# LemonATsu/UNet-PhaseGen

Measured on NVIDIA B200. Metric: audio_seconds_per_second_mag_to_phase_to_wave, higher is better.
Workload: dtype f16x3/f16x2/f16-fp32acc (two-product fp16 on d1,u2; single fp16 product = TF32 operand rounding on u1)

## Files before the change

### unet-phasegen_b200/csrc/api.cu

```cuda
#include <cstdarg>
#include <cstdio>

#include "common.cuh"
#include "conv_plan.h"

namespace pg {
static thread_local char g_err[512] = "";

void set_error(const char* fmt, ...) {
    va_list ap;
    va_start(ap, fmt);
    vsnprintf(g_err, sizeof(g_err), fmt, ap);
    va_end(ap);
}

int check_launch(const char* what) {
    cudaError_t e = cudaGetLastError();
    if (e != cudaSuccess) {
        set_error("%s: launch failed: %s", what, cudaGetErrorString(e));
        return PG_ERR_CUDA;
    }
    return PG_OK;
}
}
// ... 26 lines not shown
    pg::ConvPlan pl;
    int rc = pg::conv_plan_build(d, &pl);
    if (rc != PG_OK) return rc;
    return pl.OS * pl.n_ntiles;
}

extern "C" int pg_conv_tc_plan(const pg_conv_desc* d, int* out, int n_out) {
    PG_REQUIRE(d && out && n_out >= 16, "pg_conv_tc_plan: need a descriptor and room for 16 ints");
    pg::ConvPlan p;
    int rc = pg::conv_plan_build(d, &p);
    if (rc != PG_OK) return rc;
    const int v[16] = {p.n_tile, p.n_ntiles, p.nb, p.strip_rows, p.pair, p.merged, p.mgroups, p.acc_stages,
                       p.n_chunks, p.n_cotiles, p.OS, p.IS, p.n_taps[0], p.n_taps[1], p.n_groups[0], p.n_groups[1]};
    for (int i = 0; i < 16; ++i) out[i] = v[i];
    if (n_out >= 17) out[16] = p.whole_clip;
    return PG_OK;
}
```

### unet-phasegen_b200/csrc/conv_plan.h

```cpp
#pragma once
#include <stdint.h>
#include <stdlib.h>

#include "../../include/phasegen.h"
#include "common.cuh"

namespace pg {

constexpr int kMaxTaps = 32;

struct ConvTap { int8_t w_idx; int8_t shift; int8_t parity; int8_t pad_; int32_t d; };
struct ConvGroup { int32_t row0; int8_t parity; int8_t n_taps; int8_t first_tap; int8_t pad_; };

struct ConvPlan {
    int B, C_in, C_out, L_in, L_out, k;
    int IS, OS;
    int n_tile, n_ntiles;
    int n_chunks, n_cotiles;
    int strip_rows;
    int nb;
    int acc_stages;
    int pair;
    int mgroups;
    int merged;
    int clip_group;
    int whole_clip;
    int out_rows, out_ld;
    int n_groups[2], n_taps[2];
    ConvGroup groups[2][kMaxTaps];
    ConvTap taps[2][kMaxTaps];
};

static inline int floordiv(int a, int b) { return (a >= 0) ? a / b : -((-a + b - 1) / b); }

static inline int conv_plan_build(const pg_conv_desc* d, ConvPlan* p) {
    const int s = d->stride, k = d->k, pad = d->pad;
    if (s < 1 || s > 2 || k < 1 || k > kMaxTaps) { set_error("conv plan: stride must be 1 or 2 and k <= %d (got s=%d k=%d)", kMaxTaps, s, k); return PG_ERR_UNSUPPORTED; }
    const bool tr = d->kind == PG_CONV_TRANSPOSE;
    const int L_expect = tr ? (d->L_in - 1) * s - 2 * pad + k : (d->L_in + 2 * pad - k) / s + 1;
    const bool len_ok = tr ? (d->L_out >= L_expect && d->L_out < L_expect + s) : d->L_out == L_expect;
    if (!len_ok || d->L_out < 1) { set_error("conv plan: L_out %d does not match geometry (expected %d)", d->L_out, L_expect); return PG_ERR_INVALID; }
// ... 122 lines not shown
                const int planes = (d->precision == PG_PREC_BF16X3 || d->precision == PG_PREC_F16X3 || d->precision == PG_PREC_F16X2) ? 2 : 1;
                if (nb * p->n_ntiles * p->strip_rows * planes * 128 > 72 * 1024) nb = 1;
                if (p->n_ntiles * p->strip_rows * planes * 128 > 80 * 1024) {
                    set_error("conv plan: the %d strips of a whole clip (%d rows each) do not fit shared memory", p->n_ntiles, p->strip_rows);
                    return PG_ERR_UNSUPPORTED;
                }
                p->nb = nb;
            }
        }
    }
    {
        const int cols = p->merged ? p->nb * p->strip_rows : p->nb * p->n_tile * (p->whole_clip ? p->OS * p->n_ntiles : 1);
        if (cols > 512) { set_error("conv plan: tile needs %d accumulator columns (> 512)", cols); return PG_ERR_UNSUPPORTED; }
        p->acc_stages = cols <= 256 ? 2 : 1;
    }
    p->clip_group = d->B;
    return PG_OK;
}

}
```

### unet-phasegen_b200/csrc/conv_tc.cu

```cuda
#include "tc_ptx.cuh"
#include "conv_plan.h"

namespace pg {

struct ConvTcParams {
    ConvPlan plan;
    float* y;
    float4* stats;
    int n_a_slots;
    int b_slot_bytes;
    int n_terms;
    int f16;
    int base_offset_mode;
    int a_mn;
    int epi_mode;
    const float* gamma; const float* beta; float eps;
    ActDst dst0, dst1;
    float2* ss_out;
    const int* clip_rows;
};

constexpr int kThreads = 192;
constexpr int kATileBytes = 128 * 128;
constexpr int kMaxASlots = 8;

struct TileCoord { int co_tile, phase, b0, nt; };

__device__ __forceinline__ int n_bundles(const ConvPlan& p) { return (p.B + p.nb - 1) / p.nb; }
__device__ __forceinline__ int n_co_slabs(const ConvPlan& p) { return p.pair ? p.n_cotiles / 2 : p.n_cotiles; }
__device__ __forceinline__ int tile_OS(const ConvPlan& p) { return p.whole_clip ? 1 : p.OS; }
__device__ __forceinline__ int tile_NT(const ConvPlan& p) { return p.whole_clip ? 1 : p.n_ntiles; }
__device__ __forceinline__ int total_tiles(const ConvPlan& p) { return n_co_slabs(p) * tile_OS(p) * n_bundles(p) * tile_NT(p); }
__device__ __forceinline__ TileCoord decode_tile(const ConvPlan& p, int tile) {
    TileCoord c;
    const int OSx = tile_OS(p), NTx = tile_NT(p);
    const int nbg = n_bundles(p), G = p.clip_group, n_slabs = n_co_slabs(p) * OSx;
    const int tiles_full = n_slabs * G * NTx;
    const int g = tile / tiles_full, r = tile % tiles_full;
    int Gg = nbg - g * G; if (Gg > G) Gg = G;
    const int per_slab = Gg * NTx;
    const int slab = r / per_slab, r2 = r % per_slab;
    c.co_tile = slab / OSx; c.phase = slab % OSx;
    c.b0 = (g * G + r2 / NTx) * p.nb; c.nt = r2 % NTx;
    return c;
}

template <bool PAIR, bool RAGGED>
__global__ void __launch_bounds__(kThreads, 1)
conv_tc_kernel(const __grid_constant__ CUtensorMap map_w_hi, const __grid_constant__ CUtensorMap map_w_lo,
               const __grid_constant__ CUtensorMap map_x_hi, const __grid_constant__ CUtensorMap map_x_lo,
               const __grid_constant__ ConvTcParams prm) {
    extern __shared__ __align__(1024) uint8_t smem_raw[];
    const ConvPlan& pl = prm.plan;
    uint8_t* smem = reinterpret_cast<uint8_t*>((reinterpret_cast<uintptr_t>(smem_raw) + 1023) & ~uintptr_t(1023));
    const int nA = prm.n_a_slots;
    const int bPlane = prm.b_slot_bytes;
    const int a_planes = prm.n_terms == 3 ? 2 : 1;
    const int b_planes = prm.n_terms >= 2 ? 2 : 1;
    uint8_t* a_base = smem;
    uint8_t* b_base = a_base + (size_t)nA * a_planes * kATileBytes;
    uint64_t* bars = reinterpret_cast<uint64_t*>(b_base + 2 * (size_t)b_planes * bPlane);
    uint64_t* fullA = bars;
    uint64_t* emptyA = bars + kMaxASlots;
    uint64_t* fullB = bars + 2 * kMaxASlots;
    uint64_t* emptyB = fullB + 2;
    uint64_t* accFull = emptyB + 2;
    uint64_t* accEmpty = accFull + 2;
    uint32_t* tmem_slot = reinterpret_cast<uint32_t*>(accEmpty + 2);
    uint32_t* epi_tiles = reinterpret_cast<uint32_t*>(reinterpret_cast<uint8_t*>(bars) + 256);

    const int warp = __shfl_sync(0xffffffffu, (int)(threadIdx.x >> 5), 0), lane = threadIdx.x & 31;
    const int n_tiles = total_tiles(pl);
    const bool w_lo = prm.n_terms == 3, x_lo = prm.n_terms >= 2;

    if (warp == 0 && lane == 0) {
        tma_prefetch_desc(&map_w_hi); tma_prefetch_desc(&map_x_hi);
        if (w_lo) tma_prefetch_desc(&map_w_lo);
        if (x_lo) tma_prefetch_desc(&map_x_lo);
        for (int i = 0; i < nA; ++i) { mbar_init(fullA + i, 1); mbar_init(emptyA + i, 1); }
        for (int i = 0; i < 2; ++i) {
            mbar_init(fullB + i, 1); mbar_init(emptyB + i, 1);
            mbar_init(accFull + i, 1); mbar_init(accEmpty + i, PAIR ? 8 : 4);
        }
        fence_barrier_init();
    }
    if (warp == 1) { if (PAIR) tmem_alloc_pair(tmem_slot, 512); else tmem_alloc(tmem_slot, 512); }
    tc_fence_before();
    if (PAIR) cluster_sync_all(); else __syncthreads();
    tc_fence_after();
    const uint32_t tmem_base = __shfl_sync(0xffffffffu, *tmem_slot, 0);
    const int rank = PAIR ? (int)cluster_ctarank() : 0;
    const int tile0 = PAIR ? (int)(blockIdx.x >> 1) : (int)blockIdx.x;
    const int tile_step = PAIR ? (int)(gridDim.x >> 1) : (int)gridDim.x;
    const int half_n = pl.n_tile >> 1;
    const int nb_grp = pl.nb / pl.mgroups;
    const int nb_cta = (PAIR && pl.merged) ? nb_grp >> 1 : nb_grp;
    const int t_phases = pl.whole_clip ? pl.OS : 1;
    const int t_nts = pl.whole_clip ? pl.n_ntiles : 1;
    const int n_sub = pl.merged ? pl.mgroups : t_nts;

    if (warp == 0) {
        {
            uint32_t b_it = 0;
            int a_slot = 0; uint32_t a_ph = 0;
            const uint32_t grp_bytes = (uint32_t)nb_cta * pl.strip_rows * 128u;
            const uint32_t a_bytes = a_planes * kATileBytes;
            const uint32_t b_bytes = b_planes * (uint32_t)bPlane;
            for (int tile = tile0; tile < n_tiles; tile += tile_step) {
                TileCoord tc = decode_tile(pl, tile);
                if (PAIR) tc.co_tile = tc.co_tile * 2 + rank;
                const int m0 = tc.nt * pl.n_tile + ((PAIR && !pl.merged) ? rank * half_n : 0);
                const int clip0 = tc.b0 + ((PAIR && pl.merged) ? rank * nb_cta : 0);
                for (int ch = 0; ch < pl.n_chunks; ++ch) {
                  for (int ph = tc.phase; ph < tc.phase + t_phases; ++ph) {
                    const int ng = pl.n_groups[ph];
                    for (int g = 0; g < ng; ++g) {
                        const ConvGroup grp = pl.groups[ph][g];
                        {
                            const int s = b_it & 1; const uint32_t bph = (b_it >> 1) & 1;
                            mbar_wait(emptyB + s, bph ^ 1);
                            uint8_t* dst = b_base + (size_t)s * b_planes * bPlane;
                            if (elect_one()) {
                                if (PAIR) { if (rank == 0) mbar_expect_tx(fullB + s, 2 * b_bytes); }
                                else mbar_expect_tx(fullB + s, b_bytes);
                                for (int sub = 0; sub < n_sub; ++sub) {
                                    uint8_t* dg = dst + (size_t)sub * grp_bytes;
                                    const int cg = clip0 + (pl.merged ? sub * nb_grp : 0);
                                    const int r0 = m0 + (pl.merged ? 0 : sub * pl.n_tile) + grp.row0;
                                    if (PAIR) {
                                        tma_load_4d_pair(dg, &map_x_hi, fullB + s, ch * 64, grp.parity, r0, cg);
                                        if (x_lo) tma_load_4d_pair(dg + bPlane, &map_x_lo, fullB + s, ch * 64, grp.parity, r0, cg);
                                    } else {
                                        tma_load_4d(dg, &map_x_hi, fullB + s, ch * 64, grp.parity, r0, cg);
                                        if (x_lo) tma_load_4d(dg + bPlane, &map_x_lo, fullB + s, ch * 64, grp.parity, r0, cg);
                                    }
                                }
                            }
                            __syncwarp();
                            ++b_it;
                        }
                        for (int j = 0; j < grp.n_taps; ++j) {
                            const int w_idx = pl.taps[ph][grp.first_tap + j].w_idx;
                            const int s = a_slot; const uint32_t aph = a_ph;
                            mbar_wait(emptyA + s, aph ^ 1);
                            uint8_t* dst = a_base + (size_t)s * a_planes * kATileBytes;
                            if (elect_one()) {
                                if (!PAIR) mbar_expect_tx(fullA + s, a_bytes);
                                else if (rank == 0) mbar_expect_tx(fullA + s, 2 * a_bytes);
                                auto load_w = [&](uint8_t* d, const CUtensorMap* m, int c0, int c1) {
                                    if (PAIR) tma_load_3d_pair(d, m, fullA + s, c0, c1, w_idx);
                                    else tma_load_3d(d, m, fullA + s, c0, c1, w_idx);
                                };
                                if (prm.a_mn) {
                                    for (int h = 0; h < 2; ++h) {
                                        load_w(dst + h * 8192, &map_w_hi, tc.co_tile * 128 + h * 64, ch * 64);
                                        if (w_lo) load_w(dst + kATileBytes + h * 8192, &map_w_lo, tc.co_tile * 128 + h * 64, ch * 64);
                                    }
                                } else {
                                    load_w(dst, &map_w_hi, ch * 64, tc.co_tile * 128);
                                    if (w_lo) load_w(dst + kATileBytes, &map_w_lo, ch * 64, tc.co_tile * 128);
                                }
                            }
                            __syncwarp();
                            if (++a_slot == nA) { a_slot = 0; a_ph ^= 1; }
                        }
                    }
                  }
                }
            }
        }
    } else if (warp == 1) {
        if (rank == 0) {
            uint32_t b_it = 0, t_it = 0;
            int a_slot = 0; uint32_t a_ph = 0;
            const int n_mma = pl.merged ? nb_grp * pl.strip_rows : pl.n_tile;
            const int n_outer = pl.merged ? 1 : t_nts, n_inner = pl.merged ? pl.mgroups : pl.nb;
            const uint32_t dcol_step = pl.merged ? (uint32_t)n_mma : (uint32_t)(pl.n_tile * t_phases * t_nts);
            const uint32_t idesc = (make_idesc_bf16(n_mma, PAIR ? 256 : 128) & ~(prm.f16 ? ((7u << 7) | (7u << 10)) : 0u)) |
                                   (prm.a_mn ? (1u << 15) : 0u);
            const bool a_mn = prm.a_mn != 0;
            auto mma = [&](uint32_t d, uint32_t da, uint32_t db, uint32_t acc_flag) {
                if (elect_one()) { if (PAIR) umma_words_pair(d, da, db, idesc, acc_flag); else umma_words(d, da, db, idesc, acc_flag); }
            };
            const uint32_t a_step = a_mn ? (2048u >> 4) : (32u >> 4);
            auto commit = [&](uint64_t* bar) {
                if (elect_one()) { if (PAIR) umma_commit_pair(bar); else umma_commit(bar); }
                __syncwarp();
            };
            for (int tile = tile0; tile < n_tiles; tile += tile_step, ++t_it) {
                TileCoord tc = decode_tile(pl, tile);
                const int acc = pl.acc_stages == 2 ? (t_it & 1) : 0;
                const uint32_t acc_ph = pl.acc_stages == 2 ? ((t_it >> 1) & 1) : (t_it & 1);
                mbar_wait_sleep(accEmpty + acc, acc_ph ^ 1, 200);
                tc_fence_after();
                const uint32_t d_tmem = tmem_base + acc * 256;
                const uint32_t strip_bytes = (uint32_t)pl.strip_rows * 128u;
                const uint32_t clip_step = (pl.merged ? (uint32_t)nb_cta * strip_bytes : strip_bytes) >> 4;
                for (int ch = 0; ch < pl.n_chunks; ++ch) {
                  for (int ph = tc.phase; ph < tc.phase + t_phases; ++ph) {
                    const int ng = pl.n_groups[ph];
                    const uint32_t dcol_ph = d_tmem + (uint32_t)((ph - tc.phase) * t_nts * pl.n_tile);
                    for (int g = 0; g < ng; ++g) {
                        const ConvGroup grp = pl.groups[ph][g];
                        const int bs = b_it & 1; const uint32_t bph = (b_it >> 1) & 1;
                        mbar_wait(fullB + bs, bph);
                        tc_fence_after();
                        const uint32_t b_hi = smem_u32(b_base + (size_t)bs * b_planes * bPlane);
// ... 20 lines not shown
                                            mma(dcol, aw_hi + kk * a_step, bw_lo + kk * 2, 1);
                                            mma(dcol, aw_hi + kk * a_step, bw_hi + kk * 2, 1);
                                        }
                                    } else if (x_lo) {
#pragma unroll
                                        for (uint32_t kk = 0; kk < 4; ++kk) {
                                            mma(dcol, aw_hi + kk * a_step, bw_lo + kk * 2, kk == 0 ? acc_first : 1u);
                                            mma(dcol, aw_hi + kk * a_step, bw_hi + kk * 2, 1);
                                        }
                                    } else {
#pragma unroll
                                        for (uint32_t kk = 0; kk < 4; ++kk) mma(dcol, aw_hi + kk * a_step, bw_hi + kk * 2, kk == 0 ? acc_first : 1u);
                                    }
                                }
                            }
                            commit(emptyA + as);
                            if (++a_slot == nA) { a_slot = 0; a_ph ^= 1; }
                        }
                        commit(emptyB + bs);
                        ++b_it;
                    }
                  }
                }
                commit(accFull + acc);
            }
        }
    } else {
        const int q = warp & 3;
        uint32_t* tile = epi_tiles + q * 512;
        uint32_t t_it = 0;
        const int n_parts = t_phases * t_nts;
        const int col_pitch = pl.merged ? pl.strip_rows : pl.n_tile * n_parts;
        bool bad_range = false;
        auto store_f32 = [&](float* base, size_t off0, size_t row_pitch, const float* v, int nv) {
#pragma unroll
            for (int i = 0; i < 16; ++i) tile[i * 32 + lane] = __float_as_uint(v[i]);
            __syncwarp();
#pragma unroll
            for (int t = 0; t < 4; ++t) {
// ... 23 lines not shown
                if (r < nv) {
                    const uint4 w0 = *reinterpret_cast<const uint4*>(tile + r * 32 + part * 8);
                    const uint4 w1 = *reinterpret_cast<const uint4*>(tile + r * 32 + part * 8 + 4);
                    uint4 hv, lv;
                    hv.x = __byte_perm(w0.x, w0.y, 0x5410); hv.y = __byte_perm(w0.z, w0.w, 0x5410);
                    hv.z = __byte_perm(w1.x, w1.y, 0x5410); hv.w = __byte_perm(w1.z, w1.w, 0x5410);
                    lv.x = __byte_perm(w0.x, w0.y, 0x7632); lv.y = __byte_perm(w0.z, w0.w, 0x7632);
                    lv.z = __byte_perm(w1.x, w1.y, 0x7632); lv.w = __byte_perm(w1.z, w1.w, 0x7632);
                    const size_t o = off0 + (size_t)r * row_pitch + part * 8;
                    *reinterpret_cast<uint4*>(static_cast<uint16_t*>(d.hi) + o) = hv;
                    if (two) *reinterpret_cast<uint4*>(static_cast<uint16_t*>(d.lo) + o) = lv;
                }
            }
            __syncwarp();
        };
        for (int tile_i = tile0; tile_i < n_tiles; tile_i += tile_step, ++t_it) {
            TileCoord tc = decode_tile(pl, tile_i);
            if (PAIR) tc.co_tile = tc.co_tile * 2 + rank;
            const int acc = pl.acc_stages == 2 ? (t_it & 1) : 0;
            const uint32_t acc_ph = pl.acc_stages == 2 ? ((t_it >> 1) & 1) : (t_it & 1);
            mbar_wait_sleep(accFull + acc, acc_ph, 1000);
            tc_fence_after();
            const int co_base = tc.co_tile * 128 + q * 32;
            const int co = co_base + lane;
            auto part_geom = [&](int p, int L, int& phase, int& m0, int& n_valid) {
                phase = tc.phase + p / t_nts;
                m0 = (tc.nt + p % t_nts) * pl.n_tile;
                const int l_phase = (L - phase + pl.OS - 1) / pl.OS;
                n_valid = l_phase - m0; if (n_valid > pl.n_tile) n_valid = pl.n_tile; if (n_valid < 0) n_valid = 0;
            };
            for (int c = 0; c < pl.nb; ++c) {
                const int b = tc.b0 + c;
                if (b >= pl.B) break;
                const int L_b = RAGGED ? min(__ldg(prm.clip_rows + b), pl.L_out) : pl.L_out;
                const uint32_t tclip = tmem_base + acc * 256 + c * col_pitch + ((uint32_t)(q * 32) << 16);
                if (prm.epi_mode == PG_EPI_RAW) {
                    for (int p = 0; p < n_parts; ++p) {
                        int phase, m0, n_valid;
                        part_geom(p, L_b, phase, m0, n_valid);
                        const uint32_t taddr = tclip + p * pl.n_tile;
                        float sum = 0.f;
                        for (int c0 = 0; c0 < n_valid; c0 += 16) {
                            float v[16];
                            tmem_ld16(taddr + c0, v);
#pragma unroll
                            for (int i = 0; i < 16; ++i) if (c0 + i < n_valid) sum += v[i];
                        }
                        const float mean = n_valid > 0 ? sum / (float)n_valid : 0.f;
                        float m2 = 0.f;
                        const size_t row_pitch = (size_t)pl.OS * pl.out_ld;
// ... 75 lines not shown
                    }
                }
            }
            tc_fence_before();
            __syncwarp();
            if (lane == 0) { if (PAIR) mbar_arrive_leader(accEmpty + acc); else mbar_arrive(accEmpty + acc); }
        }
        if (bad_range) {
            if (prm.dst0.range_flag) atomicOr(prm.dst0.range_flag, 1);
            else if (prm.dst1.range_flag) atomicOr(prm.dst1.range_flag, 1);
        }
    }
    tc_fence_before();
    if (PAIR) cluster_sync_all(); else __syncthreads();
    if (warp == 1) { tc_fence_after(); if (PAIR) tmem_dealloc_pair(tmem_base, 512); else tmem_dealloc(tmem_base, 512); }
}

static EncodeTiledFn get_encode() {
    static EncodeTiledFn fn = nullptr;
    if (!fn) {
        void* p = nullptr;
        cudaDriverEntryPointQueryResult qres;
        if (cudaGetDriverEntryPoint("cuTensorMapEncodeTiled", &p, cudaEnableDefault, &qres) == cudaSuccess &&
            qres == cudaDriverEntryPointSuccess)
            fn = reinterpret_cast<EncodeTiledFn>(p);
    }
    return fn;
}

int encode_bf16_map(CUtensorMap* map, const void* base, int rank, const uint64_t* dims, const uint64_t* strides_bytes,
// ... 87 lines not shown
    prm.f16 = (d->precision == PG_PREC_F16X3 || d->precision == PG_PREC_F16X2 || d->precision == PG_PREC_F16) ? 1 : 0;
    prm.base_offset_mode = d->tc_base_offset_mode;
    prm.a_mn = d->weights_mn_major ? 1 : 0;
    const int nb_grp = pl.nb / pl.mgroups;
    const int nb_cta = (pl.pair && pl.merged) ? nb_grp / 2 : nb_grp;
    prm.b_slot_bytes = (pl.merged ? pl.mgroups : (pl.whole_clip ? pl.n_ntiles : 1)) * nb_cta * pl.strip_rows * 128;
    const int a_planes = n_terms == 3 ? 2 : 1, b_planes = n_terms >= 2 ? 2 : 1;
    const int fixed = 2 * b_planes * prm.b_slot_bytes + 1024  + 256  + 8192  +
                      (pl.merged ? 2048 : 0);
    int nA = (g_max_smem - fixed) / (a_planes * kATileBytes);
    if (nA > kMaxASlots) nA = kMaxASlots;
    PG_REQUIRE(nA >= 2, "pg_conv_tc: strip of %d rows leaves no room for the weight ring", pl.strip_rows);
    prm.n_a_slots = nA;
    const size_t smem_bytes = (size_t)fixed + (size_t)nA * a_planes * kATileBytes;

    CUtensorMap mw_hi, mw_lo, mx_hi, mx_lo;
    {
        const uint64_t inner = prm.a_mn ? d->C_out : d->C_in, outer = prm.a_mn ? d->C_in : d->C_out;
        uint64_t dims[3] = {inner, outer, (uint64_t)d->k};
        uint64_t str[2] = {inner * 2, inner * outer * 2};
        uint32_t box[3] = {64, prm.a_mn ? 64u : 128u, 1};
        if ((rc = encode_bf16_map(&mw_hi, w_hi, 3, dims, str, box, "w_hi")) != PG_OK) return rc;
        if ((rc = encode_bf16_map(&mw_lo, three ? w_lo : w_hi, 3, dims, str, box, "w_lo")) != PG_OK) return rc;
    }
    {
        const int IS = pl.IS;
        uint64_t dims[4] = {(uint64_t)d->C_in, (uint64_t)IS, (uint64_t)((d->L_in + IS - 1) / IS), (uint64_t)d->B};
        uint64_t str[3] = {(uint64_t)d->in_ld * 2, (uint64_t)d->in_ld * 2 * IS, (uint64_t)d->in_rows * d->in_ld * 2};
        uint32_t box[4] = {64, 1, (uint32_t)pl.strip_rows, (uint32_t)nb_cta};
        PG_REQUIRE(d->in_rows >= ((d->L_in + IS - 1) / IS) * IS, "pg_conv_tc: in_rows %d too small for L_in %d at stride %d", d->in_rows, d->L_in, IS);
        if ((rc = encode_bf16_map(&mx_hi, x_hi, 4, dims, str, box, "x_hi")) != PG_OK) return rc;
        if ((rc = encode_bf16_map(&mx_lo, n_terms >= 2 ? x_lo : x_hi, 4, dims, str, box, "x_lo")) != PG_OK) return rc;
    }
    const bool pair = pl.pair != 0;
    auto kernel = pair ? (ragged ? conv_tc_kernel<true, true> : conv_tc_kernel<true, false>)
                       : (ragged ? conv_tc_kernel<false, true> : conv_tc_kernel<false, false>);
    {
        static size_t configured_dev[kMaxDevices][4] = {};
        const int variant = 2 * pair + ragged;
        size_t* configured = configured_dev[current_device_slot()];
        if (smem_bytes > configured[variant]) {
            cudaError_t e = cudaFuncSetAttribute(kernel, cudaFuncAttributeMaxDynamicSharedMemorySize, (int)smem_bytes);
            if (e != cudaSuccess) { set_error("conv_tc: cannot opt in to %zu bytes of shared memory: %s", smem_bytes, cudaGetErrorString(e)); return PG_ERR_CUDA; }
            configured[variant] = smem_bytes;
        }
    }
    {
        const int nbg = (pl.B + pl.nb - 1) / pl.nb;
        const double bundle_bytes = (double)pl.nb * d->in_rows * d->in_ld * (n_terms >= 2 ? 4.0 : 2.0);
        int G = (int)(64.0e6 / bundle_bytes);
        if (const char* e = getenv("PG_TC_CLIP_GROUP")) G = atoi(e);
        if (G < 1) G = 1;
        if (G > nbg) G = nbg;
        prm.plan.clip_group = G;
    }
    const int n_tiles = (pair ? pl.n_cotiles / 2 : pl.n_cotiles) * ((pl.B + pl.nb - 1) / pl.nb) * (pl.whole_clip ? 1 : pl.OS * pl.n_ntiles);
    int units = pair ? g_sm_count / 2 : g_sm_count;
    if (const char* e = getenv("PG_TC_MAX_CTAS")) {
        const int cap = atoi(e);
        if (cap > 0 && units > (pair ? cap / 2 : cap)) units = pair ? cap / 2 : cap;
    }
    if (d->tc_max_ctas > 0 && units > (pair ? (d->tc_max_ctas + 1) / 2 : d->tc_max_ctas)) units = pair ? (d->tc_max_ctas + 1) / 2 : d->tc_max_ctas;
    if (units > n_tiles) units = n_tiles;
    cudaLaunchConfig_t cfg = {};
    cfg.gridDim = dim3(pair ? 2 * units : units);
    cfg.blockDim = dim3(kThreads);
    cfg.dynamicSmemBytes = smem_bytes;
    cfg.stream = reinterpret_cast<cudaStream_t>(stream);
    cudaLaunchAttribute attr[1];
    attr[0].id = cudaLaunchAttributeClusterDimension;
    attr[0].val.clusterDim.x = pair ? 2 : 1; attr[0].val.clusterDim.y = 1; attr[0].val.clusterDim.z = 1;
    cfg.attrs = attr; cfg.numAttrs = 1;
    cudaError_t le = cudaLaunchKernelEx(&cfg, kernel, mw_hi, mw_lo, mx_hi, mx_lo, prm);
    if (le != cudaSuccess) { set_error("conv_tc_kernel launch failed: %s", cudaGetErrorString(le)); return PG_ERR_CUDA; }
    return check_launch("conv_tc_kernel");
}

extern "C" int pg_conv_tc(const pg_conv_desc* d, const uint16_t* x_hi, const uint16_t* x_lo, const uint16_t* w_hi,
                          const uint16_t* w_lo, float* y, float* stats, const pg_conv_epilogue* epi, pg_stream stream) {
    return conv_tc_launch(d, x_hi, x_lo, w_hi, w_lo, y, stats, epi, nullptr, stream);
}

extern "C" int pg_conv_tc_ragged(const pg_conv_desc* d, const uint16_t* x_hi, const uint16_t* x_lo, const uint16_t* w_hi,
                                 const uint16_t* w_lo, float* y, float* stats, const pg_conv_epilogue* epi, const int* out_rows,
                                 pg_stream stream) {
    PG_REQUIRE(out_rows, "pg_conv_tc_ragged: null per-clip row table");
    return conv_tc_launch(d, x_hi, x_lo, w_hi, w_lo, y, stats, epi, out_rows, stream);
}
// ... 1 lines not shown
```

### unet-phasegen_b200/csrc/tc_ptx.cuh

```cuda
#pragma once
#include <cuda.h>

#include <cstdio>
#include <cstdlib>

#include "common.cuh"

namespace pg {

__device__ __forceinline__ uint32_t smem_u32(const void* p) { return (uint32_t)__cvta_generic_to_shared(p); }

__device__ __forceinline__ void mbar_init(uint64_t* bar, uint32_t count) {
    asm volatile("mbarrier.init.shared::cta.b64 [%0], %1;" ::"r"(smem_u32(bar)), "r"(count));
}
__device__ __forceinline__ void mbar_expect_tx(uint64_t* bar, uint32_t bytes) {
    asm volatile("mbarrier.arrive.expect_tx.shared::cta.b64 _, [%0], %1;" ::"r"(smem_u32(bar)), "r"(bytes) : "memory");
}
__device__ __forceinline__ void mbar_arrive(uint64_t* bar) {
    asm volatile("mbarrier.arrive.shared::cta.b64 _, [%0];" ::"r"(smem_u32(bar)) : "memory");
}
__device__ __forceinline__ bool mbar_try_wait(uint64_t* bar, uint32_t parity) {
    uint32_t ok;
    asm volatile(
        "{\n\t.reg .pred p;\n\t"
// ... 97 lines not shown
}
__device__ __forceinline__ void tmem_alloc_pair(uint32_t* dst_smem, uint32_t cols) {
    asm volatile("tcgen05.alloc.cta_group::2.sync.aligned.shared::cta.b32 [%0], %1;" ::"r"(smem_u32(dst_smem)), "r"(cols) : "memory");
    asm volatile("tcgen05.relinquish_alloc_permit.cta_group::2.sync.aligned;" ::: "memory");
}
__device__ __forceinline__ void tmem_dealloc_pair(uint32_t addr, uint32_t cols) {
    asm volatile("tcgen05.dealloc.cta_group::2.sync.aligned.b32 %0, %1;" ::"r"(addr), "r"(cols) : "memory");
}
__device__ __forceinline__ void umma_bf16_pair(uint32_t d_tmem, uint64_t a_desc, uint64_t b_desc, uint32_t idesc, uint32_t accumulate) {
    asm volatile(
        "{\n\t.reg .pred p;\n\t"
        "setp.ne.b32 p, %4, 0;\n\t"
        "tcgen05.mma.cta_group::2.kind::f16 [%0], %1, %2, %3, p;\n\t}"
        ::"r"(d_tmem), "l"(a_desc), "l"(b_desc), "r"(idesc), "r"(accumulate) : "memory");
}
__device__ __forceinline__ void umma_commit_pair(uint64_t* bar) {
    asm volatile("tcgen05.commit.cta_group::2.mbarrier::arrive::one.shared::cluster.multicast::cluster.b64 [%0], %1;"
                 ::"r"(smem_u32(bar)), "h"((uint16_t)3) : "memory");
}
__device__ __forceinline__ void mbar_arrive_leader(uint64_t* bar) {
    asm volatile("mbarrier.arrive.release.cluster.shared::cluster.b64 _, [%0];" ::"r"(smem_u32(bar) & kPeerBitMask) : "memory");
}

__device__ __forceinline__ uint64_t make_desc_sw128(uint32_t saddr, int base_offset_mode) {
    uint64_t d = 0;
    d |= (uint64_t)((saddr & 0x3FFFF) >> 4);
    d |= (uint64_t)0 << 16;
    d |= (uint64_t)(1024 >> 4) << 32;
    d |= (uint64_t)1 << 46;
    if (base_offset_mode) d |= (uint64_t)((saddr >> 7) & 7) << 49;
    d |= (uint64_t)2 << 61;
    return d;
}
constexpr uint32_t kDescHiSw128 = (1024u >> 4) | (1u << 14) | (2u << 29);
__device__ __forceinline__ uint32_t desc_lo_sw128(uint32_t saddr) { return (saddr & 0x3FFFF) >> 4; }
__device__ __forceinline__ uint32_t desc_lo_sw128_mn(uint32_t saddr, uint32_t lbo_bytes) {
// ... 49 lines not shown
```

### unet-phasegen_b200/phasegen/ops.py

```python
import ctypes as C
import math

import torch

from . import _lib
from ._lib import (ActDst, ConvDesc, ConvEpilogue, PG_EPI_ACT, PG_EPI_NORM_ACT, PG_EPI_RAW, PG_CONV, PG_CONV_TRANSPOSE, PG_DT_BF16, PG_DT_BF16_SPLIT, PG_DT_F16,
                   PG_DT_F16_SPLIT, PG_DT_F32, PG_DT_NONE, PG_FMT_BF16, PG_FMT_F16, PG_PREC_BF16, PG_PREC_BF16X3,
                   PG_PREC_F16X2, PG_PREC_F16X3, PG_PREC_FP32_SIMT, PG_SPEC_CARTESIAN, PG_SPEC_POLAR_LOG,
                   PG_SPEC_POLAR_MAG, PG_STFT_LOGMAG, PG_STFT_REIM)

SUPPORTED_N_FFT = (256, 512, 1024, 2048)


def _stream(t=None):
    dev = t.device if isinstance(t, torch.Tensor) and t.is_cuda else None
    return C.c_void_p(torch.cuda.current_stream(dev).cuda_stream)


def _ptr(t):
    return C.c_void_p(t.data_ptr()) if t is not None else C.c_void_p(0)


def _fmt(t):
    if t is None or t.dtype == torch.bfloat16:
# ... 179 lines not shown
def conv_epilogue_supported(desc, mode):
    r = _lib.load().pg_conv_epilogue_supported(C.byref(desc), mode)
    if r < 0:
        raise RuntimeError(f"pg_conv_epilogue_supported failed ({r}): {_lib.last_error()}")
    return bool(r)


def conv_stat_parts(desc):
    p = _lib.load().pg_conv_stat_parts(C.byref(desc))
    if p <= 0:
        raise RuntimeError(f"pg_conv_stat_parts failed ({p}): {_lib.last_error()}")
    return p


_PLAN_KEYS = ("n_tile", "n_ntiles", "nb", "strip_rows", "pair", "merged", "mgroups", "acc_stages", "n_chunks", "n_cotiles",
              "OS", "IS", "taps0", "taps1", "groups0", "groups1", "whole_clip")


def conv_plan(desc, whole_clip=None):
    d = ConvDesc.from_buffer_copy(desc)
    if whole_clip is not None:
        d.tc_whole_clip = int(whole_clip)
    out = (C.c_int * 17)()
    if _lib.load().pg_conv_tc_plan(C.byref(d), out, 17) != 0:
        return None
    pl = dict(zip(_PLAN_KEYS, out))
    slabs = pl["n_cotiles"] // 2 if pl["pair"] else pl["n_cotiles"]
    parts = 1 if pl["whole_clip"] else pl["OS"] * pl["n_ntiles"]
    pl["tiles"] = slabs * parts * -(-d.B // pl["nb"])
    pl["units"] = 74 if pl["pair"] else 148
    return pl


def conv_simt(desc, x, w_simt, y):
    _lib.call("pg_conv_simt", C.byref(desc), _ptr(x), _ptr(w_simt), _ptr(y), _stream())


def channel_stats(y, B, L, Cn, rows, ld, stats):
    _lib.call("pg_channel_stats", _ptr(y), B, L, Cn, rows, ld, _ptr(stats), _stream())
# ... 90 lines not shown
```

Measured before the change: 45960.

## Add 4-CTA cluster mode with weight multicast and dynamic tile scheduling to conv kernel

Adds a 'quad' mode for paired tensor-core convolutions. It asks for a preferred cluster size of 4 so that two CTA pairs share weight tiles through TMA multicast, with each pair loading half the weights. In the split variant each pair handles one clip, using the smem freed for extra A slots and a second accumulator stage. Tiles are now claimed dynamically through a global atomic counter that is broadcast across the cluster via mbarriers, replacing static striding. This cuts redundant weight traffic and balances load, but adds cross-CTA synchronisation, atomic scheduling overhead and deadlock or timeout risk.

```diff
diff --git a/unet-phasegen_b200/csrc/api.cu b/unet-phasegen_b200/csrc/api.cu
--- a/unet-phasegen_b200/csrc/api.cu
+++ b/unet-phasegen_b200/csrc/api.cu
@@ -64,5 +64,6 @@
                        p.n_chunks, p.n_cotiles, p.OS, p.IS, p.n_taps[0], p.n_taps[1], p.n_groups[0], p.n_groups[1]};
     for (int i = 0; i < 16; ++i) out[i] = v[i];
     if (n_out >= 17) out[16] = p.whole_clip;
+    if (n_out >= 18) out[17] = p.quad;
     return PG_OK;
 }
diff --git a/unet-phasegen_b200/csrc/conv_plan.h b/unet-phasegen_b200/csrc/conv_plan.h
--- a/unet-phasegen_b200/csrc/conv_plan.h
+++ b/unet-phasegen_b200/csrc/conv_plan.h
@@ -25,6 +25,7 @@
     int merged;
     int clip_group;
     int whole_clip;
+    int quad;
     int out_rows, out_ld;
     int n_groups[2], n_taps[2];
     ConvGroup groups[2][kMaxTaps];
@@ -177,6 +178,14 @@
         if (cols > 512) { set_error("conv plan: tile needs %d accumulator columns (> 512)", cols); return PG_ERR_UNSUPPORTED; }
         p->acc_stages = cols <= 256 ? 2 : 1;
     }
+    p->quad = 0;
+    if (p->pair && !p->merged && !d->weights_mn_major) {
+        if (p->acc_stages == 1 && d->precision == PG_PREC_F16X2 && p->nb == 2 && !p->whole_clip) p->quad = 1;
+        else p->quad = 2;
+    }
+    if (const char* e = getenv("PG_TC_CLUSTER")) {
+        if (atoi(e) == 2) p->quad = 0;
+    }
     p->clip_group = d->B;
     return PG_OK;
 }
diff --git a/unet-phasegen_b200/csrc/conv_tc.cu b/unet-phasegen_b200/csrc/conv_tc.cu
--- a/unet-phasegen_b200/csrc/conv_tc.cu
+++ b/unet-phasegen_b200/csrc/conv_tc.cu
@@ -18,11 +18,15 @@
     ActDst dst0, dst1;
     float2* ss_out;
     const int* clip_rows;
+    int sched_slot;
 };
 
 constexpr int kThreads = 192;
 constexpr int kATileBytes = 128 * 128;
 constexpr int kMaxASlots = 8;
+
+constexpr int kSchedSlots = 64;
+__device__ unsigned int g_conv_sched[kSchedSlots][2];
 
 struct TileCoord { int co_tile, phase, b0, nt; };
 
@@ -49,17 +53,32 @@
 __global__ void __launch_bounds__(kThreads, 1)
 conv_tc_kernel(const __grid_constant__ CUtensorMap map_w_hi, const __grid_constant__ CUtensorMap map_w_lo,
                const __grid_constant__ CUtensorMap map_x_hi, const __grid_constant__ CUtensorMap map_x_lo,
-               const __grid_constant__ ConvTcParams prm) {
+               const __grid_constant__ CUtensorMap map_w_half, const __grid_constant__ CUtensorMap map_w_half_lo,
+               const __grid_constant__ CUtensorMap map_x1_hi,
+               const __grid_constant__ CUtensorMap map_x1_lo, const __grid_constant__ ConvTcParams prm) {
     extern __shared__ __align__(1024) uint8_t smem_raw[];
     const ConvPlan& pl = prm.plan;
     uint8_t* smem = reinterpret_cast<uint8_t*>((reinterpret_cast<uintptr_t>(smem_raw) + 1023) & ~uintptr_t(1023));
-    const int nA = prm.n_a_slots;
-    const int bPlane = prm.b_slot_bytes;
+    const uint32_t ncta = PAIR ? cluster_nctarank() : 1u;
+    const bool quad = PAIR && ncta == 4;
+    const bool split = quad && pl.quad == 1;
+    const bool tpair = PAIR && pl.quad == 2;
+    const bool dyn = PAIR && pl.quad;
+    const uint32_t crank = PAIR ? cluster_ctarank() : 0u;
+    const int rank = (int)(crank & 1u);
+    const int pr = (int)(crank >> 1);
     const int a_planes = prm.n_terms == 3 ? 2 : 1;
     const int b_planes = prm.n_terms >= 2 ? 2 : 1;
+    const int bPlane = split ? prm.b_slot_bytes / 2 : prm.b_slot_bytes;
+    int nA = prm.n_a_slots;
+    if (split) {
+        nA += (2 * b_planes * bPlane) / (a_planes * kATileBytes);
+        if (nA > kMaxASlots) nA = kMaxASlots;
+    }
     uint8_t* a_base = smem;
     uint8_t* b_base = a_base + (size_t)nA * a_planes * kATileBytes;
-    uint64_t* bars = reinterpret_cast<uint64_t*>(b_base + 2 * (size_t)b_planes * bPlane);
+    uint64_t* bars = reinterpret_cast<uint64_t*>(smem + (size_t)prm.n_a_slots * a_planes * kATileBytes +
+                                                 2 * (size_t)b_planes * prm.b_slot_bytes);
     uint64_t* fullA = bars;
     uint64_t* emptyA = bars + kMaxASlots;
     uint64_t* fullB = bars + 2 * kMaxASlots;
@@ -67,6 +86,9 @@
     uint64_t* accFull = emptyB + 2;
     uint64_t* accEmpty = accFull + 2;
     uint32_t* tmem_slot = reinterpret_cast<uint32_t*>(accEmpty + 2);
+    uint64_t* schedFull = accEmpty + 3;
+    uint64_t* schedEmpty = schedFull + 2;
+    int* sched_tile = reinterpret_cast<int*>(schedEmpty + 2);
     uint32_t* epi_tiles = reinterpret_cast<uint32_t*>(reinterpret_cast<uint8_t*>(bars) + 256);
 
     const int warp = __shfl_sync(0xffffffffu, (int)(threadIdx.x >> 5), 0), lane = threadIdx.x & 31;
@@ -74,13 +96,14 @@
     const bool w_lo = prm.n_terms == 3, x_lo = prm.n_terms >= 2;
 
     if (warp == 0 && lane == 0) {
-        tma_prefetch_desc(&map_w_hi); tma_prefetch_desc(&map_x_hi);
-        if (w_lo) tma_prefetch_desc(&map_w_lo);
-        if (x_lo) tma_prefetch_desc(&map_x_lo);
-        for (int i = 0; i < nA; ++i) { mbar_init(fullA + i, 1); mbar_init(emptyA + i, 1); }
+        tma_prefetch_desc(quad ? &map_w_half : &map_w_hi); tma_prefetch_desc(split ? &map_x1_hi : &map_x_hi);
+        if (w_lo) tma_prefetch_desc(quad ? &map_w_half_lo : &map_w_lo);
+        if (x_lo) tma_prefetch_desc(split ? &map_x1_lo : &map_x_lo);
+        for (int i = 0; i < nA; ++i) { mbar_init(fullA + i, 1); mbar_init(emptyA + i, quad ? 2 : 1); }
         for (int i = 0; i < 2; ++i) {
             mbar_init(fullB + i, 1); mbar_init(emptyB + i, 1);
             mbar_init(accFull + i, 1); mbar_init(accEmpty + i, PAIR ? 8 : 4);
+            mbar_init(schedFull + i, 1); mbar_init(schedEmpty + i, 5 * ncta + ncta / 2);
         }
         fence_barrier_init();
     }
@@ -89,15 +112,45 @@
     if (PAIR) cluster_sync_all(); else __syncthreads();
     tc_fence_after();
     const uint32_t tmem_base = __shfl_sync(0xffffffffu, *tmem_slot, 0);
-    const int rank = PAIR ? (int)cluster_ctarank() : 0;
     const int tile0 = PAIR ? (int)(blockIdx.x >> 1) : (int)blockIdx.x;
     const int tile_step = PAIR ? (int)(gridDim.x >> 1) : (int)gridDim.x;
+    const int acc_stages = split ? 2 : pl.acc_stages;
     const int half_n = pl.n_tile >> 1;
     const int nb_grp = pl.nb / pl.mgroups;
     const int nb_cta = (PAIR && pl.merged) ? nb_grp >> 1 : nb_grp;
     const int t_phases = pl.whole_clip ? pl.OS : 1;
     const int t_nts = pl.whole_clip ? pl.n_ntiles : 1;
     const int n_sub = pl.merged ? pl.mgroups : t_nts;
+    unsigned int* sched = g_conv_sched[prm.sched_slot];
+    auto next_unit = [&](uint32_t k, bool fetch) -> int {
+        const int s = (int)(k & 1u); const uint32_t ph = (k >> 1) & 1u;
+        if (fetch) {
+            mbar_wait_cluster(schedEmpty + s, ph ^ 1u);
+            if (lane == 0) {
+                const uint32_t t = atomicAdd(sched, 1u);
+                for (uint32_t r = 0; r < ncta; ++r) {
+                    st_cluster_u32(map_rank(sched_tile + s, r), t);
+                    mbar_arrive_remote(map_rank(schedFull + s, r));
+                }
+            }
+            __syncwarp();
+        }
+        mbar_wait_cluster(schedFull + s, ph);
+        int t = 0;
+        if (lane == 0) {
+            t = *reinterpret_cast<volatile int*>(sched_tile + s);
+            mbar_arrive_remote(map_rank(schedEmpty + s, 0));
+        }
+        return __shfl_sync(0xffffffffu, t, 0);
+    };
+    const uint32_t pair_seq = (tpair && !quad) ? 1u : 0u;
+    int unit = 0;
+    auto tile_at = [&](uint32_t it, bool fetch) -> int {
+        if (!dyn) return tile0 + (int)it * tile_step;
+        const uint32_t j = it & pair_seq, k = it >> pair_seq;
+        if (j == 0) unit = next_unit(k, fetch);
+        return tpair ? 2 * unit + (quad ? pr : (int)j) : unit;
+    };
 
     if (warp == 0) {
         {
@@ -106,11 +159,17 @@
             const uint32_t grp_bytes = (uint32_t)nb_cta * pl.strip_rows * 128u;
             const uint32_t a_bytes = a_planes * kATileBytes;
             const uint32_t b_bytes = b_planes * (uint32_t)bPlane;
-            for (int tile = tile0; tile < n_tiles; tile += tile_step) {
+            const CUtensorMap* mx_hi = split ? &map_x1_hi : &map_x_hi;
+            const CUtensorMap* mx_lo = split ? &map_x1_lo : &map_x_lo;
+            const uint32_t w_mask = (1u << rank) | (4u << rank);
+            const bool fetch = dyn && crank == 0;
+            for (uint32_t it = 0;; ++it) {
+                const int tile = tile_at(it, fetch);
+                if (tile >= n_tiles) break;
                 TileCoord tc = decode_tile(pl, tile);
                 if (PAIR) tc.co_tile = tc.co_tile * 2 + rank;
                 const int m0 = tc.nt * pl.n_tile + ((PAIR && !pl.merged) ? rank * half_n : 0);
-                const int clip0 = tc.b0 + ((PAIR && pl.merged) ? rank * nb_cta : 0);
+                const int clip0 = tc.b0 + ((PAIR && pl.merged) ? rank * nb_cta : 0) + (split ? pr : 0);
                 for (int ch = 0; ch < pl.n_chunks; ++ch) {
                   for (int ph = tc.phase; ph < tc.phase + t_phases; ++ph) {
                     const int ng = pl.n_groups[ph];
@@ -128,8 +187,8 @@
                                     const int cg = clip0 + (pl.merged ? sub * nb_grp : 0);
                                     const int r0 = m0 + (pl.merged ? 0 : sub * pl.n_tile) + grp.row0;
                                     if (PAIR) {
-                                        tma_load_4d_pair(dg, &map_x_hi, fullB + s, ch * 64, grp.parity, r0, cg);
-                                        if (x_lo) tma_load_4d_pair(dg + bPlane, &map_x_lo, fullB + s, ch * 64, grp.parity, r0, cg);
+                                        tma_load_4d_pair(dg, mx_hi, fullB + s, ch * 64, grp.parity, r0, cg);
+                                        if (x_lo) tma_load_4d_pair(dg + bPlane, mx_lo, fullB + s, ch * 64, grp.parity, r0, cg);
                                     } else {
                                         tma_load_4d(dg, &map_x_hi, fullB + s, ch * 64, grp.parity, r0, cg);
                                         if (x_lo) tma_load_4d(dg + bPlane, &map_x_lo, fullB + s, ch * 64, grp.parity, r0, cg);
@@ -151,7 +210,12 @@
                                     if (PAIR) tma_load_3d_pair(d, m, fullA + s, c0, c1, w_idx);
                                     else tma_load_3d(d, m, fullA + s, c0, c1, w_idx);
                                 };
-                                if (prm.a_mn) {
+                                if (quad) {
+                                    tma_load_3d_pair_mc(dst + pr * 8192, &map_w_half, fullA + s, w_mask, ch * 64,
+                                                        tc.co_tile * 128 + pr * 64, w_idx);
+                                    if (w_lo) tma_load_3d_pair_mc(dst + kATileBytes + pr * 8192, &map_w_half_lo, fullA + s, w_mask,
+                                                                  ch * 64, tc.co_tile * 128 + pr * 64, w_idx);
+                                } else if (prm.a_mn) {
                                     for (int h = 0; h < 2; ++h) {
                                         load_w(dst + h * 8192, &map_w_hi, tc.co_tile * 128 + h * 64, ch * 64);
                                         if (w_lo) load_w(dst + kATileBytes + h * 8192, &map_w_lo, tc.co_tile * 128 + h * 64, ch * 64);
@@ -174,7 +238,7 @@
             uint32_t b_it = 0, t_it = 0;
             int a_slot = 0; uint32_t a_ph = 0;
             const int n_mma = pl.merged ? nb_grp * pl.strip_rows : pl.n_tile;
-            const int n_outer = pl.merged ? 1 : t_nts, n_inner = pl.merged ? pl.mgroups : pl.nb;
+            const int n_outer = pl.merged ? 1 : t_nts, n_inner = pl.merged ? pl.mgroups : split ? 1 : pl.nb;
             const uint32_t dcol_step = pl.merged ? (uint32_t)n_mma : (uint32_t)(pl.n_tile * t_phases * t_nts);
             const uint32_t idesc = (make_idesc_bf16(n_mma, PAIR ? 256 : 128) & ~(prm.f16 ? ((7u << 7) | (7u << 10)) : 0u)) |
                                    (prm.a_mn ? (1u << 15) : 0u);
@@ -183,14 +247,17 @@
                 if (elect_one()) { if (PAIR) umma_words_pair(d, da, db, idesc, acc_flag); else umma_words(d, da, db, idesc, acc_flag); }
             };
             const uint32_t a_step = a_mn ? (2048u >> 4) : (32u >> 4);
-            auto commit = [&](uint64_t* bar) {
-                if (elect_one()) { if (PAIR) umma_commit_pair(bar); else umma_commit(bar); }
+            const uint32_t pair_mask = 3u << (2 * pr), a_mask = quad ? 0xFu : pair_mask;
+            auto commit = [&](uint64_t* bar, uint32_t mask) {
+                if (elect_one()) { if (PAIR) umma_commit_pair(bar, mask); else umma_commit(bar); }
                 __syncwarp();
             };
-            for (int tile = tile0; tile < n_tiles; tile += tile_step, ++t_it) {
+            for (;; ++t_it) {
+                const int tile = tile_at(t_it, false);
+                if (tile >= n_tiles) break;
                 TileCoord tc = decode_tile(pl, tile);
-                const int acc = pl.acc_stages == 2 ? (t_it & 1) : 0;
-                const uint32_t acc_ph = pl.acc_stages == 2 ? ((t_it >> 1) & 1) : (t_it & 1);
+                const int acc = acc_stages == 2 ? (t_it & 1) : 0;
+                const uint32_t acc_ph = acc_stages == 2 ? ((t_it >> 1) & 1) : (t_it & 1);
                 mbar_wait_sleep(accEmpty + acc, acc_ph ^ 1, 200);
                 tc_fence_after();
                 const uint32_t d_tmem = tmem_base + acc * 256;
@@ -241,15 +308,15 @@
                                     }
                                 }
                             }
-                            commit(emptyA + as);
+                            commit(emptyA + as, a_mask);
                             if (++a_slot == nA) { a_slot = 0; a_ph ^= 1; }
                         }
-                        commit(emptyB + bs);
+                        commit(emptyB + bs, pair_mask);
                         ++b_it;
                     }
                   }
                 }
-                commit(accFull + acc);
+                commit(accFull + acc, pair_mask);
             }
         }
     } else {
@@ -303,11 +370,14 @@
             }
             __syncwarp();
         };
-        for (int tile_i = tile0; tile_i < n_tiles; tile_i += tile_step, ++t_it) {
+        const int c_lo = split ? pr : 0, c_hi = split ? pr + 1 : pl.nb;
+        for (;; ++t_it) {
+            const int tile_i = tile_at(t_it, false);
+            if (tile_i >= n_tiles) break;
             TileCoord tc = decode_tile(pl, tile_i);
             if (PAIR) tc.co_tile = tc.co_tile * 2 + rank;
-            const int acc = pl.acc_stages == 2 ? (t_it & 1) : 0;
-            const uint32_t acc_ph = pl.acc_stages == 2 ? ((t_it >> 1) & 1) : (t_it & 1);
+            const int acc = acc_stages == 2 ? (t_it & 1) : 0;
+            const uint32_t acc_ph = acc_stages == 2 ? ((t_it >> 1) & 1) : (t_it & 1);
             mbar_wait_sleep(accFull + acc, acc_ph, 1000);
             tc_fence_after();
             const int co_base = tc.co_tile * 128 + q * 32;
@@ -318,11 +388,11 @@
                 const int l_phase = (L - phase + pl.OS - 1) / pl.OS;
                 n_valid = l_phase - m0; if (n_valid > pl.n_tile) n_valid = pl.n_tile; if (n_valid < 0) n_valid = 0;
             };
-            for (int c = 0; c < pl.nb; ++c) {
+            for (int c = c_lo; c < c_hi; ++c) {
                 const int b = tc.b0 + c;
                 if (b >= pl.B) break;
                 const int L_b = RAGGED ? min(__ldg(prm.clip_rows + b), pl.L_out) : pl.L_out;
-                const uint32_t tclip = tmem_base + acc * 256 + c * col_pitch + ((uint32_t)(q * 32) << 16);
+                const uint32_t tclip = tmem_base + acc * 256 + (c - c_lo) * col_pitch + ((uint32_t)(q * 32) << 16);
                 if (prm.epi_mode == PG_EPI_RAW) {
                     for (int p = 0; p < n_parts; ++p) {
                         int phase, m0, n_valid;
@@ -428,6 +498,10 @@
     tc_fence_before();
     if (PAIR) cluster_sync_all(); else __syncthreads();
     if (warp == 1) { tc_fence_after(); if (PAIR) tmem_dealloc_pair(tmem_base, 512); else tmem_dealloc(tmem_base, 512); }
+    if (dyn && threadIdx.x == 0) {
+        __threadfence();
+        if (atomicAdd(sched + 1, 1u) == gridDim.x - 1) { atomicExch(sched, 0u); atomicExch(sched + 1, 0u); }
+    }
 }
 
 static EncodeTiledFn get_encode() {
@@ -545,7 +619,7 @@
     prm.n_a_slots = nA;
     const size_t smem_bytes = (size_t)fixed + (size_t)nA * a_planes * kATileBytes;
 
-    CUtensorMap mw_hi, mw_lo, mx_hi, mx_lo;
+    CUtensorMap mw_hi, mw_lo, mx_hi, mx_lo, mw_half, mw_half_lo, mx1_hi, mx1_lo;
     {
         const uint64_t inner = prm.a_mn ? d->C_out : d->C_in, outer = prm.a_mn ? d->C_in : d->C_out;
         uint64_t dims[3] = {inner, outer, (uint64_t)d->k};
@@ -553,6 +627,10 @@
         uint32_t box[3] = {64, prm.a_mn ? 64u : 128u, 1};
         if ((rc = encode_bf16_map(&mw_hi, w_hi, 3, dims, str, box, "w_hi")) != PG_OK) return rc;
         if ((rc = encode_bf16_map(&mw_lo, three ? w_lo : w_hi, 3, dims, str, box, "w_lo")) != PG_OK) return rc;
+        mw_half = mw_hi; mw_half_lo = mw_lo;
+        box[1] = 64;
+        if (pl.quad && (rc = encode_bf16_map(&mw_half, w_hi, 3, dims, str, box, "w_half")) != PG_OK) return rc;
+        if (pl.quad && three && (rc = encode_bf16_map(&mw_half_lo, w_lo, 3, dims, str, box, "w_half_lo")) != PG_OK) return rc;
     }
     {
         const int IS = pl.IS;
@@ -562,6 +640,12 @@
         PG_REQUIRE(d->in_rows >= ((d->L_in + IS - 1) / IS) * IS, "pg_conv_tc: in_rows %d too small for L_in %d at stride %d", d->in_rows, d->L_in, IS);
         if ((rc = encode_bf16_map(&mx_hi, x_hi, 4, dims, str, box, "x_hi")) != PG_OK) return rc;
         if ((rc = encode_bf16_map(&mx_lo, n_terms >= 2 ? x_lo : x_hi, 4, dims, str, box, "x_lo")) != PG_OK) return rc;
+        mx1_hi = mx_hi; mx1_lo = mx_lo;
+        box[3] = 1;
+        if (pl.quad == 1 && nb_cta > 1) {
+            if ((rc = encode_bf16_map(&mx1_hi, x_hi, 4, dims, str, box, "x1_hi")) != PG_OK) return rc;
+            if ((rc = encode_bf16_map(&mx1_lo, n_terms >= 2 ? x_lo : x_hi, 4, dims, str, box, "x1_lo")) != PG_OK) return rc;
+        }
     }
     const bool pair = pl.pair != 0;
     auto kernel = pair ? (ragged ? conv_tc_kernel<true, true> : conv_tc_kernel<true, false>)
@@ -583,6 +667,10 @@
         if (const char* e = getenv("PG_TC_CLIP_GROUP")) G = atoi(e);
         if (G < 1) G = 1;
         if (G > nbg) G = nbg;
+        if (pl.quad == 2 && (pl.whole_clip ? 1 : pl.n_ntiles) % 2) {
+            if (nbg % 2) prm.plan.quad = 0;
+            else if (G % 2) G = G > 1 ? G - 1 : 2;
+        }
         prm.plan.clip_group = G;
     }
     const int n_tiles = (pair ? pl.n_cotiles / 2 : pl.n_cotiles) * ((pl.B + pl.nb - 1) / pl.nb) * (pl.whole_clip ? 1 : pl.OS * pl.n_ntiles);
@@ -593,16 +681,28 @@
     }
     if (d->tc_max_ctas > 0 && units > (pair ? (d->tc_max_ctas + 1) / 2 : d->tc_max_ctas)) units = pair ? (d->tc_max_ctas + 1) / 2 : d->tc_max_ctas;
     if (units > n_tiles) units = n_tiles;
+    const bool quad = pl.quad && units >= 2;
+    if (quad) units &= ~1;
+    if (pl.quad) {
+        static int next_slot[kMaxDevices] = {};
+        int& ns = next_slot[current_device_slot()];
+        prm.sched_slot = ns;
+        ns = (ns + 1) % kSchedSlots;
+    } else {
+        prm.sched_slot = 0;
+    }
     cudaLaunchConfig_t cfg = {};
     cfg.gridDim = dim3(pair ? 2 * units : units);
     cfg.blockDim = dim3(kThreads);
     cfg.dynamicSmemBytes = smem_bytes;
     cfg.stream = reinterpret_cast<cudaStream_t>(stream);
-    cudaLaunchAttribute attr[1];
+    cudaLaunchAttribute attr[2];
     attr[0].id = cudaLaunchAttributeClusterDimension;
     attr[0].val.clusterDim.x = pair ? 2 : 1; attr[0].val.clusterDim.y = 1; attr[0].val.clusterDim.z = 1;
-    cfg.attrs = attr; cfg.numAttrs = 1;
-    cudaError_t le = cudaLaunchKernelEx(&cfg, kernel, mw_hi, mw_lo, mx_hi, mx_lo, prm);
+    attr[1].id = cudaLaunchAttributePreferredClusterDimension;
+    attr[1].val.preferredClusterDim.x = 4; attr[1].val.preferredClusterDim.y = 1; attr[1].val.preferredClusterDim.z = 1;
+    cfg.attrs = attr; cfg.numAttrs = quad ? 2 : 1;
+    cudaError_t le = cudaLaunchKernelEx(&cfg, kernel, mw_hi, mw_lo, mx_hi, mx_lo, mw_half, mw_half_lo, mx1_hi, mx1_lo, prm);
     if (le != cudaSuccess) { set_error("conv_tc_kernel launch failed: %s", cudaGetErrorString(le)); return PG_ERR_CUDA; }
     return check_launch("conv_tc_kernel");
 }
diff --git a/unet-phasegen_b200/csrc/tc_ptx.cuh b/unet-phasegen_b200/csrc/tc_ptx.cuh
--- a/unet-phasegen_b200/csrc/tc_ptx.cuh
+++ b/unet-phasegen_b200/csrc/tc_ptx.cuh
@@ -135,12 +135,53 @@
         "tcgen05.mma.cta_group::2.kind::f16 [%0], %1, %2, %3, p;\n\t}"
         ::"r"(d_tmem), "l"(a_desc), "l"(b_desc), "r"(idesc), "r"(accumulate) : "memory");
 }
-__device__ __forceinline__ void umma_commit_pair(uint64_t* bar) {
+__device__ __forceinline__ void umma_commit_pair(uint64_t* bar, uint32_t cta_mask = 3u) {
     asm volatile("tcgen05.commit.cta_group::2.mbarrier::arrive::one.shared::cluster.multicast::cluster.b64 [%0], %1;"
-                 ::"r"(smem_u32(bar)), "h"((uint16_t)3) : "memory");
+                 ::"r"(smem_u32(bar)), "h"((uint16_t)cta_mask) : "memory");
 }
 __device__ __forceinline__ void mbar_arrive_leader(uint64_t* bar) {
     asm volatile("mbarrier.arrive.release.cluster.shared::cluster.b64 _, [%0];" ::"r"(smem_u32(bar) & kPeerBitMask) : "memory");
+}
+
+__device__ __forceinline__ uint32_t cluster_nctarank() { uint32_t n; asm volatile("mov.u32 %0, %%cluster_nctarank;" : "=r"(n)); return n; }
+__device__ __forceinline__ uint32_t map_rank(const void* p, uint32_t rank) {
+    uint32_t r;
+    asm volatile("mapa.shared::cluster.u32 %0, %1, %2;" : "=r"(r) : "r"(smem_u32(p)), "r"(rank));
+    return r;
+}
+__device__ __forceinline__ void st_cluster_u32(uint32_t addr, uint32_t v) {
+    asm volatile("st.shared::cluster.u32 [%0], %1;" ::"r"(addr), "r"(v) : "memory");
+}
+__device__ __forceinline__ void mbar_arrive_remote(uint32_t addr) {
+    asm volatile("mbarrier.arrive.release.cluster.shared::cluster.b64 _, [%0];" ::"r"(addr) : "memory");
+}
+__device__ __forceinline__ void mbar_wait_cluster(uint64_t* bar, uint32_t parity) {
+    auto try_wait = [&]() {
+        uint32_t ok;
+        asm volatile(
+            "{\n\t.reg .pred p;\n\t"
+            "mbarrier.try_wait.parity.acquire.cluster.shared::cta.b64 p, [%1], %2;\n\t"
+            "selp.u32 %0, 1, 0, p;\n\t}"
+            : "=r"(ok) : "r"(smem_u32(bar)), "r"(parity) : "memory");
+        return ok != 0;
+    };
+    if (try_wait()) return;
+    const long long t0 = clock64();
+    for (uint32_t spins = 1; !try_wait(); ++spins) {
+        if ((spins & 1023u) == 0 && clock64() - t0 > 4000000000ll) {
+            printf("phasegen conv_tc: cluster mbarrier timeout (block %d thread %d bar %u parity %u)\n",
+                   (int)blockIdx.x, (int)threadIdx.x, smem_u32(bar), parity);
+            __trap();
+        }
+    }
+}
+__device__ __forceinline__ void tma_load_3d_pair_mc(void* dst, const CUtensorMap* map, uint64_t* bar, uint32_t cta_mask,
+                                                    int c0, int c1, int c2) {
+    asm volatile(
+        "cp.async.bulk.tensor.3d.cta_group::2.shared::cluster.global.mbarrier::complete_tx::bytes.multicast::cluster"
+        " [%0], [%1, {%4, %5, %6}], [%2], %3;"
+        ::"r"(smem_u32(dst)), "l"(map), "r"(smem_u32(bar) & kPeerBitMask), "h"((uint16_t)cta_mask), "r"(c0), "r"(c1), "r"(c2)
+        : "memory");
 }
 
 __device__ __forceinline__ uint64_t make_desc_sw128(uint32_t saddr, int base_offset_mode) {
diff --git a/unet-phasegen_b200/phasegen/ops.py b/unet-phasegen_b200/phasegen/ops.py
--- a/unet-phasegen_b200/phasegen/ops.py
+++ b/unet-phasegen_b200/phasegen/ops.py
@@ -217,15 +217,15 @@
 
 
 _PLAN_KEYS = ("n_tile", "n_ntiles", "nb", "strip_rows", "pair", "merged", "mgroups", "acc_stages", "n_chunks", "n_cotiles",
-              "OS", "IS", "taps0", "taps1", "groups0", "groups1", "whole_clip")
+              "OS", "IS", "taps0", "taps1", "groups0", "groups1", "whole_clip", "quad")
 
 
 def conv_plan(desc, whole_clip=None):
     d = ConvDesc.from_buffer_copy(desc)
     if whole_clip is not None:
         d.tc_whole_clip = int(whole_clip)
-    out = (C.c_int * 17)()
-    if _lib.load().pg_conv_tc_plan(C.byref(d), out, 17) != 0:
+    out = (C.c_int * 18)()
+    if _lib.load().pg_conv_tc_plan(C.byref(d), out, 18) != 0:
         return None
     pl = dict(zip(_PLAN_KEYS, out))
     slabs = pl["n_cotiles"] // 2 if pl["pair"] else pl["n_cotiles"]
```

Result: no change. 46100 (median of 6 runs) (+0.3%).
